# avianphysics/avian

Hardware: NVIDIA H100
Metric: physics steps/sec on 100k-cube stack (broad phase + solver stage per step) (higher is better)
Workload: dtype f32

## Files before the change

### avian_b200/csrc/broadphase.cu

```cuda
#include <algorithm>
#include <cmath>
#include <cstdlib>
#include <cstring>
#include <vector>

#include "avn_math.cuh"
#include "context.hpp"

#include "device_prims.cuh"

namespace avn {
namespace {

template <class S> struct KeyOf;
template <> struct KeyOf<float> { using type = uint32_t; static constexpr int passes = 4; };
template <> struct KeyOf<double> { using type = uint64_t; static constexpr int passes = 8; };

__device__ __forceinline__ uint32_t sortable(float f) {
    uint32_t b = __float_as_uint(f);
    if (b == 0x80000000u) b = 0;
    return (b & 0x80000000u) ? ~b : (b | 0x80000000u);
}
__device__ __forceinline__ uint64_t sortable(double f) {
    uint64_t b = (uint64_t)__double_as_longlong(f);
// ... 143 lines not shown
        if (!EMIT && threadIdx.x == 0) sub_counts[w * nsub + sub] = total;
    }
}
__global__ void wide_finish(const int* __restrict__ wide_list, const int* __restrict__ wide_count, uint32_t* __restrict__ sub_counts, int nsub,
                            uint32_t* __restrict__ counts) {
    const int nw = min(*wide_count, SW_WIDE_CAP);
    for (int w = blockIdx.x * blockDim.x + threadIdx.x; w < nw; w += gridDim.x * blockDim.x) {
        uint32_t run = 0;
        for (int k = 0; k < nsub; ++k) {
            uint32_t c = sub_counts[w * nsub + k];
            sub_counts[w * nsub + k] = run;
            run += c;
        }
        counts[wide_list[w]] = run;
    }
}

}
}
#include "broadphase_cells.cuh"
namespace avn {
namespace {

template <class S>
class Broadphase final : public BroadphaseBase {
    using K = typename KeyOf<S>::type;

   public:
    Broadphase(cudaStream_t stream, ErrorSink* err, int device) : stream_(stream), err_(err) {
        cudaDeviceProp prop;
        if (cudaGetDeviceProperties(&prop, device) == cudaSuccess) sm_count_ = prop.multiProcessorCount;
        cudaEventCreate(&ev0_);
        cudaEventCreate(&ev1_);
        cudaHostAlloc(&h_total_, 2 * sizeof(uint64_t), cudaHostAllocDefault);
        const char* g = getenv("AVN_BP_GRAPH");
        use_graph_ = !(g && !strcmp(g, "0"));
    }
    ~Broadphase() override {
        cudaEventDestroy(ev0_);
        cudaEventDestroy(ev1_);
        if (h_total_) cudaFreeHost(h_total_);
        if (graph_exec_) cudaGraphExecDestroy(graph_exec_);
    }
    AvnStatus upload(AvnAabbColumns* a) override;
    AvnStatus run() override;
    AvnStatus download(AvnPairList* out) override;
    AvnStatus device_pairs(DevicePairs* out) override;
    AvnStatus download_order(uint64_t* out_pair_count) override;
    void set_existing_device(const uint64_t* table, uint64_t mask) override { ext_existing_ = table; ext_existing_mask_ = mask; }
    void timings(AvnTimings* t) const override { *t = tm_; }

   private:
    template <class T> AvnStatus up(DevBuf& buf, const void* host, size_t count, const T** dev) {
        *dev = nullptr;
        if (!host || count == 0) return AVN_OK;
        AVN_CUDA(buf.ensure(count * sizeof(T)));
        AVN_CUDA(cudaMemcpyAsync(buf.p, host, count * sizeof(T), cudaMemcpyHostToDevice, stream_));
        *dev = buf.as<T>();
        return AVN_OK;
    }
    AvnStatus build_set(DevBuf& keys_buf, DevBuf& table_buf, const uint64_t* host_keys, uint64_t count, const uint64_t** table, uint64_t* mask);
    static constexpr int WIDE_ROWS = 64;
    uint32_t graph_replays_ = 0;
    Sweep<S> sweep_desc() const {
        Sweep<S> sw;
        sw.n = n_; sw.minx = s_minx_.as<S>(); sw.maxx = s_maxx_.as<S>(); sw.yz = s_yz_.as<Vec4<S>>(); sw.meta = s_meta_.as<uint4>();
        sw.flags = s_flags_.as<uint8_t>(); sw.end = s_end_.as<int>(); sw.is_wide = wide_flag_.as<uint8_t>();
        sw.existing = d_existing_; sw.existing_mask = existing_mask_; sw.jdis = d_jdis_; sw.jdis_mask = jdis_mask_;
        return sw;
    }
    CellSweep<S> cell_desc() const {
        CellSweep<S> cs;
        cs.grid = grid_.as<CellGrid<S>>(); cs.cranks = cv0_.as<uint32_t>(); cs.cstart = cbounds_.as<int>(); cs.cend = cbounds_.as<int>() + 0x10000;
        cs.capacity = pair_capacity_;
        return cs;
    }
    AvnStatus ensure_buffers(int n);
    void enqueue_front(int n);
    AvnStatus drop_nonfinite();
    AvnStatus settle();
    AvnStatus finish_download();
    const uint64_t* ext_existing_ = nullptr; uint64_t ext_existing_mask_ = 0;

    struct GraphKey {
        int n = -1;
        const void* p[24] = {};
        uint64_t m[2] = {};
        bool operator==(const GraphKey& o) const { return n == o.n && !memcmp(p, o.p, sizeof p) && !memcmp(m, o.m, sizeof m); }
    };
    GraphKey graph_key() const;
    bool use_graph_ = true;
    cudaGraphExec_t graph_exec_ = nullptr;
    GraphKey graph_key_{};
    uint32_t front_launches_ = 0;
    DevBuf nf_flag_;
    bool dropped_ = false;
    std::vector<uint32_t> keep_;
    std::vector<unsigned char> c_min_, c_max_;
    std::vector<uint32_t> c_col_, c_body_, c_memb_, c_filt_;
    std::vector<uint8_t> c_flags_;

    cudaStream_t stream_;
    ErrorSink* err_;
    int sm_count_ = 132;
    cudaEvent_t ev0_, ev1_;
    uint64_t* h_total_ = nullptr;
    AvnTimings tm_{};
    uint32_t launches_ = 0, upload_launches_ = 0;
    bool uploaded_ = false, ran_ = false;
    int n_ = 0;
    uint64_t pair_capacity_ = 0;
    AvnAabbColumns host_{};
    AvnAabbColumns* caller_ = nullptr;
    const S* d_min_ = nullptr; const S* d_max_ = nullptr;
    const uint32_t* d_collider_ = nullptr; const uint32_t* d_body_ = nullptr; const uint32_t* d_memb_ = nullptr; const uint32_t* d_filt_ = nullptr;
    const uint8_t* d_flags_ = nullptr;
    const uint64_t* d_existing_ = nullptr; uint64_t existing_mask_ = 0;
    const uint64_t* d_jdis_ = nullptr; uint64_t jdis_mask_ = 0;
    DevBuf b_min_, b_max_, b_col_, b_body_, b_memb_, b_filt_, b_flags_, b_exk_, b_ext_, b_jdk_, b_jdt_;
    DevBuf k0_, k1_, v0_, v1_, hist_;
    DevBuf s_minx_, s_maxx_, s_yz_, s_meta_, s_flags_, s_end_, counts_, offsets_, block_sums_, wide_, wide_sub_, wide_flag_, grid_, ck0_, ck1_, cv0_, cv1_, cbounds_, pairs_, stats_, stats2_;
    DevBuf o_c1_, o_c2_, o_b1_, o_b2_, o_fl_;
    uint32_t* d_order_ = nullptr;
};

template <class S>
AvnStatus Broadphase<S>::build_set(DevBuf& keys_buf, DevBuf& table_buf, const uint64_t* host_keys, uint64_t count, const uint64_t** table, uint64_t* mask) {
    *table = nullptr;
    *mask = 0;
    if (!host_keys || count == 0) return AVN_OK;
    uint64_t cap = 64;
    while (cap < count * 2) cap <<= 1;
    const uint64_t* dkeys;
    AvnStatus st = up<uint64_t>(keys_buf, host_keys, count, &dkeys);
    if (st != AVN_OK) return st;
// ... 57 lines not shown
    AVN_CUDA(wide_.ensure((size_t(SW_WIDE_CAP) + 1) * 4));
    AVN_CUDA(wide_flag_.ensure(size_t(n)));
    const int nsub = (n + SW_SUB - 1) / SW_SUB;
    AVN_CUDA(wide_sub_.ensure(size_t(nsub) * size_t(std::min(n, SW_WIDE_CAP)) * 4));
    AVN_CUDA(block_sums_.ensure(size_t((n + 1023) / 1024) * 8));
    AVN_CUDA(nf_flag_.ensure(8));
    pair_capacity_ = std::max<uint64_t>(pair_capacity_, uint64_t(4) * uint64_t(n) + 1024);
    AVN_CUDA(o_c1_.ensure(pair_capacity_ * 4)); AVN_CUDA(o_c2_.ensure(pair_capacity_ * 4)); AVN_CUDA(o_b1_.ensure(pair_capacity_ * 4)); AVN_CUDA(o_b2_.ensure(pair_capacity_ * 4));
    AVN_CUDA(o_fl_.ensure(pair_capacity_));
    AVN_CUDA(pairs_.ensure(pair_capacity_ * sizeof(uint2)));
    return AVN_OK;
}

template <class S>
typename Broadphase<S>::GraphKey Broadphase<S>::graph_key() const {
    GraphKey k;
    k.n = n_;
    const void* ptrs[] = {d_min_, d_max_, d_collider_, d_body_, d_memb_, d_filt_, d_flags_, d_existing_, d_jdis_, k0_.p, k1_.p, v0_.p, v1_.p, hist_.p,
                          s_minx_.p, s_maxx_.p, s_yz_.p, s_meta_.p, s_flags_.p, s_end_.p, counts_.p, offsets_.p, grid_.p, ck0_.p};
    static_assert(sizeof ptrs == sizeof k.p, "graph key size");
    memcpy(k.p, ptrs, sizeof ptrs);
    k.m[0] = existing_mask_ ^ (uint64_t(uintptr_t(cv0_.p)) << 1) ^ (uint64_t(uintptr_t(wide_sub_.p)) << 2);
    k.m[0] ^= (pair_capacity_ * 0x9e3779b97f4a7c15ull) ^ (uint64_t(uintptr_t(pairs_.p)) << 3) ^ (uint64_t(uintptr_t(o_c1_.p)) << 4) ^ (uint64_t(uintptr_t(o_fl_.p)) << 5);
    k.m[1] = jdis_mask_ ^ (uint64_t(uintptr_t(cbounds_.p)) << 1) ^ (uint64_t(uintptr_t(block_sums_.p)) << 2) ^ (uint64_t(uintptr_t(wide_flag_.p)) << 3);
    return k;
}

template <class S>
void Broadphase<S>::enqueue_front(int n) {
    const int nblocks = (n + RS_TILE - 1) / RS_TILE;
    uint32_t launches = 0;
    K* ka = k0_.as<K>(); K* kb = k1_.as<K>();
    uint32_t* va = v0_.as<uint32_t>(); uint32_t* vb = v1_.as<uint32_t>();
    cudaMemsetAsync(nf_flag_.p, 0, 8, stream_);
    make_keys<S><<<(n + 255) / 256, 256, 0, stream_>>>(d_min_, d_max_, n, ka, va, nf_flag_.as<unsigned long long>());
    ++launches;
    for (int pass = 0; pass < KeyOf<S>::passes; ++pass) {
        const int shift = 8 * pass;
        rs_histogram<K><<<nblocks, RS_THREADS, 0, stream_>>>(ka, n, shift, hist_.as<uint32_t>(), nblocks);
        if (nblocks <= RS_FUSE_MAX_BLOCKS) {
            rs_scatter<K, true><<<nblocks, RS_THREADS, 0, stream_>>>(ka, va, n, shift, hist_.as<uint32_t>(), nblocks, kb, vb);
        } else {
            rs_scan<<<1, 1024, 0, stream_>>>(hist_.as<uint32_t>(), 256 * nblocks);
            rs_scatter<K, false><<<nblocks, RS_THREADS, 0, stream_>>>(ka, va, n, shift, hist_.as<uint32_t>(), nblocks, kb, vb);
        }
        launches += nblocks <= RS_FUSE_MAX_BLOCKS ? 2 : 3;
        std::swap(ka, kb);
        std::swap(va, vb);
    }
    d_order_ = va;
    gather_sorted<S><<<(n + 255) / 256, 256, 0, stream_>>>(d_order_, n, d_min_, d_max_, d_collider_, d_body_, d_memb_, d_filt_, d_flags_,
                                                           s_minx_.as<S>(), s_maxx_.as<S>(), s_yz_.as<Vec4<S>>(), s_meta_.as<uint4>(),
                                                           s_flags_.as<uint8_t>());
    CellGrid<S>* d_grid = grid_.as<CellGrid<S>>();
    int* cstart = cbounds_.as<int>();
    int* cend = cbounds_.as<int>() + 0x10000;
    yz_stats<S><<<YZ_BLOCKS, 256, 0, stream_>>>(s_yz_.as<Vec4<S>>(), n, stats_.as<YzPartial<S>>());
    yz_fold<S><<<1, 32, 0, stream_>>>(stats_.as<YzPartial<S>>(), YZ_BLOCKS, n, d_grid);
    yz_small_max<S><<<YZ_BLOCKS, 256, 0, stream_>>>(s_yz_.as<Vec4<S>>(), n, d_grid, stats2_.as<S>());
    yz_grid<S><<<1, 32, 0, stream_>>>(stats_.as<YzPartial<S>>(), stats2_.as<S>(), YZ_BLOCKS, n, d_grid);
    int* wide_count = wide_.as<int>();
    int* wide_list = wide_.as<int>() + 1;
    cudaMemsetAsync(wide_count, 0, 4, stream_);
    sweep_bounds<S><<<(n + 255) / 256, 256, 0, stream_>>>(s_minx_.as<S>(), s_maxx_.as<S>(), s_yz_.as<Vec4<S>>(), d_grid, n, s_end_.as<int>(), wide_list, wide_count,
                                                          wide_flag_.as<uint8_t>(), s_flags_.as<uint8_t>());
    const Sweep<S> sw = sweep_desc();
    cell_keys<S><<<(n + 255) / 256, 256, 0, stream_>>>(s_yz_.as<Vec4<S>>(), n, d_grid, ck0_.as<uint32_t>(), cv0_.as<uint32_t>());
    {
        uint32_t* cka = ck0_.as<uint32_t>(); uint32_t* ckb = ck1_.as<uint32_t>();
        uint32_t* cva = cv0_.as<uint32_t>(); uint32_t* cvb = cv1_.as<uint32_t>();
        for (int pass = 0; pass < 2; ++pass) {
            rs_histogram<uint32_t><<<nblocks, RS_THREADS, 0, stream_>>>(cka, n, 8 * pass, hist_.as<uint32_t>(), nblocks);
            if (nblocks <= RS_FUSE_MAX_BLOCKS) {
                rs_scatter<uint32_t, true><<<nblocks, RS_THREADS, 0, stream_>>>(cka, cva, n, 8 * pass, hist_.as<uint32_t>(), nblocks, ckb, cvb);
            } else {
                rs_scan<<<1, 1024, 0, stream_>>>(hist_.as<uint32_t>(), 256 * nblocks);
                rs_scatter<uint32_t, false><<<nblocks, RS_THREADS, 0, stream_>>>(cka, cva, n, 8 * pass, hist_.as<uint32_t>(), nblocks, ckb, cvb);
            }
            std::swap(cka, ckb);
            std::swap(cva, cvb);
        }
    }
    cudaMemsetAsync(cstart, 0x7f, size_t(0x10000) * 4, stream_);
    cudaMemsetAsync(cend, 0, size_t(0x10000) * 4, stream_);
    cell_bounds<<<(n + 255) / 256, 256, 0, stream_>>>(ck0_.as<uint32_t>(), n, cstart, cend);
    const CellSweep<S> cs = cell_desc();
    const int grid = std::min((n + (256 / CG_GROUP) - 1) / (256 / CG_GROUP), sm_count_ * 32);
    sweep_cells_kernel<S, false><<<grid, 256, 0, stream_>>>(sw, cs, counts_.as<uint32_t>(), nullptr, nullptr);
    const int nsub = (n + SW_SUB - 1) / SW_SUB;
    sweep_wide_kernel<S, false><<<dim3(nsub, WIDE_ROWS), SW_THREADS, 0, stream_>>>(sw, wide_list, wide_count, wide_sub_.as<uint32_t>(), nsub, nullptr, nullptr, 0);
    wide_finish<<<1, 256, 0, stream_>>>(wide_list, wide_count, wide_sub_.as<uint32_t>(), nsub, counts_.as<uint32_t>());
    launches += nblocks <= RS_FUSE_MAX_BLOCKS ? 15 : 17;
    const int sblocks = (n + 1023) / 1024;
    scan_block_sums<<<sblocks, 1024, 0, stream_>>>(counts_.as<uint32_t>(), n, block_sums_.as<uint64_t>());
    scan_block_offsets<<<1, 1024, 0, stream_>>>(block_sums_.as<uint64_t>(), sblocks, offsets_.as<uint64_t>() + n);
    scan_apply<<<sblocks, 1024, 0, stream_>>>(counts_.as<uint32_t>(), n, block_sums_.as<uint64_t>(), offsets_.as<uint64_t>());
    launches += 3;
    {
        uint2* pairs = pairs_.as<uint2>();
        sweep_cells_kernel<S, true><<<grid, 256, 0, stream_>>>(sw, cs, nullptr, offsets_.as<uint64_t>(), pairs);
        sweep_wide_kernel<S, true><<<dim3(nsub, WIDE_ROWS), SW_THREADS, 0, stream_>>>(sw, wide_list, wide_count, wide_sub_.as<uint32_t>(), nsub,
                                                                                      offsets_.as<uint64_t>(), pairs, pair_capacity_);
        segment_sort<<<(n + 255) / 256, 256, 0, stream_>>>(offsets_.as<uint64_t>(), wide_flag_.as<uint8_t>(), n, pairs, pair_capacity_);
        const unsigned mblocks = unsigned(std::min<uint64_t>((pair_capacity_ + 255) / 256, uint64_t(sm_count_) * 16));
        materialize_pairs<S><<<mblocks, 256, 0, stream_>>>(sw, pairs, offsets_.as<uint64_t>() + n, pair_capacity_, o_c1_.as<uint32_t>(), o_c2_.as<uint32_t>(),
                                                           o_b1_.as<uint32_t>(), o_b2_.as<uint32_t>(), o_fl_.as<uint8_t>());
        launches += 4;
    }
    cudaMemcpyAsync(h_total_, offsets_.as<uint64_t>() + n, sizeof(uint64_t), cudaMemcpyDeviceToHost, stream_);
    cudaMemcpyAsync(h_total_ + 1, nf_flag_.p, sizeof(uint64_t), cudaMemcpyDeviceToHost, stream_);
    front_launches_ = launches;
}

template <class S>
AvnStatus Broadphase<S>::run() {
    if (!uploaded_) return err_->fail(AVN_ERR_INVALID_ARGUMENT, "avn_broadphase_run before avn_broadphase_upload");
    const int n = n_;
    launches_ = upload_launches_;
    cudaEventRecord(ev0_, stream_);
    h_total_[0] = 0;
    h_total_[1] = 0;
    if (n > 0) {
        AvnStatus st = ensure_buffers(n);
        if (st != AVN_OK) return st;
        if (use_graph_) {
            const GraphKey key = graph_key();
            if (!graph_exec_ || !(key == graph_key_)) {
                if (graph_exec_) { cudaGraphExecDestroy(graph_exec_); graph_exec_ = nullptr; }
                cudaGraph_t g = nullptr;
                AVN_CUDA(cudaStreamBeginCapture(stream_, cudaStreamCaptureModeThreadLocal));
                enqueue_front(n);
                cudaError_t ce = cudaStreamEndCapture(stream_, &g);
                if (ce == cudaSuccess) ce = cudaGraphInstantiate(&graph_exec_, g, 0);
                if (g) cudaGraphDestroy(g);
                if (ce != cudaSuccess) {
// ... 156 lines not shown
```

### avian_b200/csrc/solver_dev.cuh

```cuda
#pragma once
#include <cuda_pipeline.h>

#include "../../include/avian_b200.h"
#include "avn_math.cuh"

namespace avn {

enum { CP_N = 0, CP_T1 = 1, CP_TV = 2, CP_IDX = 3, CP_PT0 = 4, CP_PLANES = CP_PT0 + 3 * AVN_MAX_MANIFOLD_POINTS };
#define CP_ROW(k, r) (CP_PT0 + 3 * (k) + (r))
enum { CI_NP_MASK = 0x7, CI_ZERO1 = 1 << 4, CI_ZERO2 = 1 << 5, CI_NONDYN = 1 << 6, CI_TANGENT = 1 << 7,
       CI_VER1 = 1 << 8, CI_VER2 = 1 << 9 };
enum { BF_LOCK_MASK = 0x3f, BF_HAS_SOLVER_BODY = 1 << 8, BF_KINEMATIC = 1 << 9, BF_GYRO = 1 << 10, BF_DYNAMIC = 1 << 11,
       BF_CUSTOM_VEL = 1 << 12, BF_CUSTOM_POS = 1 << 13, BF_DOMINANCE_SHIFT = 16 };

enum { JP_IDX = 0,
       JP_R1 = 1,
       JP_R2 = 2,
       JP_CD = 3,
       JP_RD = 4,
       JP_A1 = 5,
       JP_A2 = 6,
       JP_B1 = 7,
       JP_B2 = 8,
       JP_LP = 9,
       JP_LA = 10,
       JP_LB = 11,
       JP_PLANES = 12 };

template <class S>
struct Soft { S bias, mass_scale, impulse_scale; };

template <class S>
struct DevSolver {
    int B, M, P, Mpad, J, Jpad, n_levels, n_damp_levels;
    int m_color_off[AVN_GRAPH_COLOR_COUNT + 1];
    int color_off[AVN_GRAPH_COLOR_COUNT + 1];
    int color_len[AVN_GRAPH_COLOR_COUNT];
    int wave;
    unsigned int* ver;
    int* deg;
    int* stamp;
    int substeps, iters, rest_iters, fast_trig, match_contacts;
    S h, dt, max_overlap_speed, warm_coeff, rest_threshold, joint_force_rhs;
    S gx, gy, gz;
    Soft<S> soft_dyn, soft_nondyn;
    const uint8_t* kind; const uint8_t* locked; const int8_t* dominance; const uint8_t* integ_flags;
    const S* position; const S* rotation; const S* linvel; const S* angvel; const S* inv_mass; const S* inv_inertia_local;
    const S* com; const S* lin_damp; const S* ang_damp; const S* grav_scale; const S* lin_acc; const S* ang_acc;
    const S* max_lin; const S* max_ang;
    S* out_position; S* out_rotation; S* out_linvel; S* out_angvel;
    Vec4<S>* vel; Vec4<S>* dlt; Vec4<S>* inr; Vec4<S>* itg; Vec4<S>* pre;
    const int* m_body1; const int* m_body2; const S* m_normal; const S* m_friction; const S* m_restitution; const S* m_tanvel;
    const uint32_t* m_point_begin; const uint32_t* m_point_end; const uint32_t* m_src;
    const S* p_anchor1; const S* p_anchor2; const S* p_penetration; const S* p_normal_speed;
    const S* p_ws_normal; const S* p_ws_tangent;
    const S* p_in_normal_impulse;
    S* p_out_ws_normal; S* p_out_ws_tangent; S* p_normal_impulse;
    Vec4<S>* cst;
    Vec4<S>* pcr;
    int* any_restitution;
    const int* j_src_type; const int* j_src_index;
    const int* level_off;
    Vec4<S>* jnt;
    const S* jc[AVN_JOINT_TYPE_COUNT][12];
    const S* jdamp_lin[AVN_JOINT_TYPE_COUNT]; const S* jdamp_ang[AVN_JOINT_TYPE_COUNT];
    const uint8_t* jlimit_en[AVN_JOINT_TYPE_COUNT]; const uint8_t* jdamp_en[AVN_JOINT_TYPE_COUNT];
    const int* jbody1[AVN_JOINT_TYPE_COUNT]; const int* jbody2[AVN_JOINT_TYPE_COUNT];
    S* jforce[AVN_JOINT_TYPE_COUNT]; S* jtorque[AVN_JOINT_TYPE_COUNT];
    const int* jdamp_slot; const int* damp_level_off;
    Vec4<S>* jdummy;
    int do_prepare, sub_begin, sub_end, do_restitution, do_finalize;
    const int* bnd_of;
    Vec4<S>* vel_ref;
};
// ... 593 lines not shown
        st4(&d.vel[2 * b2 + 1], mk4<S>(w2.x, w2.y, w2.z, S(0)));
    }
    wave_publish(d.ver, ver1, b1, e1, ver2, b2, e2);
#ifdef AVN_WAVE_TRACE
    AVN_TRACE_ADD(d, 3, clock64() - t_s0);
    AVN_TRACE_ADD(d, 4, 1);
#endif
#undef ROW_A
#undef ROW_B
#undef ROW_D
#undef ROW_PC
}

template <class S, bool WAVE = false>
__device__ __forceinline__ void integrate_velocity_item(const DevSolver<S>& d, int i, int s = 0) {
    const bool in_range = i < d.B;
    int f = 0;
    if (in_range) f = as_int(ld4(&d.inr[2 * i]).y);
    const bool live = in_range && (f & BF_HAS_SOLVER_BODY);
    const bool integrate = live && !(f & BF_CUSTOM_VEL) && !(f & BF_KINEMATIC), gyro = integrate && (f & BF_GYRO);
    Vec4<S> li = mk4<S>(0, 0, 0, 0), ai = li;
    Q4<S> rot0; rot0.x = rot0.y = rot0.z = rot0.w = S(0);
    Sym3<S> il; il.m00 = il.m01 = il.m02 = il.m11 = il.m12 = il.m22 = S(0);
    if (integrate) { li = ld4(&d.itg[2 * i]); ai = ld4(&d.itg[2 * i + 1]); }
    if (gyro) {
        rot0 = ldq(d.rotation, i);
        il.m00 = d.inv_inertia_local[6 * i]; il.m01 = d.inv_inertia_local[6 * i + 1]; il.m02 = d.inv_inertia_local[6 * i + 2];
        il.m11 = d.inv_inertia_local[6 * i + 3]; il.m12 = d.inv_inertia_local[6 * i + 4]; il.m22 = d.inv_inertia_local[6 * i + 5];
    }
    const S max_lin = live && d.max_lin ? d.max_lin[i] : S(0), max_ang = live && d.max_ang ? d.max_ang[i] : S(0);
    const int bnd = live && d.bnd_of ? d.bnd_of[i] : -1;
    unsigned e = 0;
    if (WAVE) {
        if (live) e = wave_event(WV_IV, 0, s, d.iters, d.deg[i], 0);
        wave_wait(d.ver, live, i, e, false, 0, 0u, d.any_restitution + 1);
    }
    if (!live) return;
    Vec4<S> l = ldm<WAVE>(&d.vel[2 * i]), a = ldm<WAVE>(&d.vel[2 * i + 1]);
    V3<S> v = xyz(l), w = xyz(a);
    bool touched = false;
    if (integrate) {
        v = v * li.w;
        w = w * ai.w;
        v = v + xyz(li);
        w = w + xyz(ai);
        if (gyro) {
            Vec4<S> dq4 = ldm<WAVE>(&d.dlt[2 * i + 1]);
            Q4<S> dq; dq.x = dq4.x; dq.y = dq4.y; dq.z = dq4.z; dq.w = dq4.w;
            Q4<S> rot = qmul(dq, rot0);
            V3<S> lw = qrot(qconj(rot), w);
            Sym3<S> tensor = sym_inverse_or_zero(il);
            V3<S> L = smul(tensor, lw);
            V3<S> Ln = L - d.h * cross(lw, L);
            S l2 = len2(Ln);
            if (l2 == S(0)) {
                w = zero3<S>();
            } else {
                Ln = Ln * avn_sqrt(len2(L) / l2);
                w = qrot(rot, smul(il, Ln));
            }
        }
        touched = true;
    }
    if (d.max_lin) {
        S l2 = len2(v);
        if (avn_finite(max_lin) && l2 > max_lin * max_lin) { v = v * (max_lin / avn_sqrt(l2)); touched = true; }
    }
    if (d.max_ang) {
        S l2 = len2(w);
        if (avn_finite(max_ang) && l2 > max_ang * max_ang) { w = w * (max_ang / avn_sqrt(l2)); touched = true; }
    }
    if (touched) {
        st4(&d.vel[2 * i], mk4<S>(v.x, v.y, v.z, S(0)));
        st4(&d.vel[2 * i + 1], mk4<S>(w.x, w.y, w.z, S(0)));
    }
    if (bnd >= 0) {
        st4(&d.vel_ref[2 * bnd], mk4<S>(v.x, v.y, v.z, S(0)));
        st4(&d.vel_ref[2 * bnd + 1], mk4<S>(w.x, w.y, w.z, S(0)));
    }
    if (WAVE) wave_publish(d.ver, true, i, e, false, 0, 0u);
}

template <class S, bool WAVE = false>
__device__ __forceinline__ void integrate_position_item(const DevSolver<S>& d, int i, int s = 0) {
    const bool in_range = i < d.B;
    int f = 0;
    if (in_range) f = as_int(ld4(&d.inr[2 * i]).y);
    const bool live = in_range && (f & BF_HAS_SOLVER_BODY);
    unsigned e = 0;
    if (WAVE) {
        if (live) e = wave_event(WV_IP, 0, s, d.iters, d.deg[i], 0);
        wave_wait(d.ver, live, i, e, false, 0, 0u, d.any_restitution + 1);
    }
    if (!live) return;
    if (f & BF_CUSTOM_POS) {
        if (WAVE) wave_publish(d.ver, true, i, e, false, 0, 0u);
        return;
    }
    Vec4<S> l = ldm<WAVE>(&d.vel[2 * i]), a = ldm<WAVE>(&d.vel[2 * i + 1]);
    Vec4<S> dp = ldm<WAVE>(&d.dlt[2 * i]), dq4 = ldm<WAVE>(&d.dlt[2 * i + 1]);
    V3<S> ndp = xyz(dp) + xyz(l) * d.h;
    Q4<S> dq; dq.x = dq4.x; dq.y = dq4.y; dq.z = dq4.z; dq.w = dq4.w;
    Q4<S> nq = qmul(q_from_scaled_axis(xyz(a) * d.h, d.fast_trig != 0), dq);
    st4(&d.dlt[2 * i], mk4<S>(ndp.x, ndp.y, ndp.z, S(0)));
    st4(&d.dlt[2 * i + 1], mk4<S>(nq.x, nq.y, nq.z, nq.w));
    if (WAVE) wave_publish(d.ver, true, i, e, false, 0, 0u);
}

enum { WAVE_WATCHDOG = 1, WAVE_BAD_COLOURING = 3 };
template <class S>
__device__ __forceinline__ void wave_rank_item(const DevSolver<S>& d, int slot) {
    const size_t MP = size_t(d.Mpad);
    Vec4<S>* c = d.cst + slot;
    Vec4<S> hidx = ld4(&c[CP_IDX * MP]);
    const int info = as_int(hidx.z);
    if ((info & CI_NP_MASK) == 0) return;
    const int b1 = as_int(hidx.x), b2 = as_int(hidx.y);
    int colour = 0;
    while (colour < AVN_GRAPH_COLOR_COUNT - 1 && slot >= d.color_off[colour + 1]) ++colour;
    int r1 = 0, r2 = 0;
    bool bad = false;
    if (info & CI_VER1) { bad |= atomicExch(&d.stamp[b1], colour + 1) == colour + 1; r1 = atomicAdd(&d.deg[b1], 1); }
    if (info & CI_VER2) { bad |= atomicExch(&d.stamp[b2], colour + 1) == colour + 1; r2 = atomicAdd(&d.deg[b2], 1); }
    if (bad || r1 > 0xfe || r2 > 0xfe) d.any_restitution[1] = WAVE_BAD_COLOURING;
    hidx.w = int_as(S(0), (r1 & 0xff) | ((r2 & 0xff) << 16));
    st4(&c[CP_IDX * MP], hidx);
}
template <class S>
__device__ __forceinline__ void wave_pack_item(const DevSolver<S>& d, int slot) {
    const size_t MP = size_t(d.Mpad);
    Vec4<S>* c = d.cst + slot;
    Vec4<S> hidx = ld4(&c[CP_IDX * MP]);
    const int info = as_int(hidx.z);
    if ((info & CI_NP_MASK) == 0) return;
    const int b1 = as_int(hidx.x), b2 = as_int(hidx.y);
    int rk = as_int(hidx.w);
    if (info & CI_VER1) rk |= (d.deg[b1] & 0xff) << 8;
    if (info & CI_VER2) rk |= (d.deg[b2] & 0xff) << 24;
    hidx.w = int_as(S(0), rk);
    st4(&c[CP_IDX * MP], hidx);
}

template <class S>
__device__ __forceinline__ void writeback_body_item(const DevSolver<S>& d, int i) {
    Vec4<S> ia = ld4(&d.inr[2 * i]);
    int f = as_int(ia.y);
    V3<S> pos = ldv3(d.position, i);
    Q4<S> rot = ldq(d.rotation, i);
    V3<S> lv = ldv3(d.linvel, i), av = ldv3(d.angvel, i);
    if (f & BF_HAS_SOLVER_BODY) {
        Vec4<S> l = ld4(&d.vel[2 * i]), a = ld4(&d.vel[2 * i + 1]);
        Vec4<S> dp = ld4(&d.dlt[2 * i]), dq4 = ld4(&d.dlt[2 * i + 1]);
        V3<S> com = ldv3_or0(d.com, i);
        V3<S> old_com = qrot(rot, com);
        Q4<S> dq; dq.x = dq4.x; dq.y = dq4.y; dq.z = dq4.z; dq.w = dq4.w;
        rot = q_fast_renormalize(qmul(dq, rot));
        V3<S> new_com = qrot(rot, com);
        pos = pos + ((xyz(dp) + old_com) - new_com);
        lv = xyz(l);
        av = xyz(a);
    }
    stv3(d.out_position, i, pos);
    d.out_rotation[4 * i] = rot.x; d.out_rotation[4 * i + 1] = rot.y; d.out_rotation[4 * i + 2] = rot.z; d.out_rotation[4 * i + 3] = rot.w;
    stv3(d.out_linvel, i, lv);
    stv3(d.out_angvel, i, av);
}

template <class S>
__device__ __forceinline__ void store_impulse_item(const DevSolver<S>& d, int m) {
    const size_t MP = size_t(d.Mpad);
    const int slot = slot_of_manifold(d, m);
// ... 23 lines not shown
```

### avian_b200/csrc/solver_host.cu

```cuda
#include <algorithm>
#include <cmath>
#include <cstdlib>
#include <cstring>

#include "context.hpp"
#include "joint_schedule.hpp"
#include "solver_kernels.cuh"

namespace avn {

namespace {

template <class S>
Soft<S> softness(S damping_ratio, S hz, S delta_secs) {
    S double_damping_ratio = S(2) * damping_ratio;
    S angular_frequency = S(6.283185307179586476925286766559) * hz;
    S a1 = double_damping_ratio + angular_frequency * delta_secs;
    S a2 = angular_frequency * delta_secs * a1;
    S a3 = S(1) / (S(1) + a2);
    Soft<S> s;
    s.bias = angular_frequency / a1;
    s.mass_scale = a2 * a3;
    s.impulse_scale = a3;
    return s;
// ... 446 lines not shown
            d.p_ws_normal = static_cast<const S*>(mc->ws_normal); d.p_ws_tangent = static_cast<const S*>(mc->ws_tangent);
            d.p_in_normal_impulse = static_cast<const S*>(mc->normal_impulse);
            d.p_out_ws_normal = static_cast<S*>(mc->out_ws_normal); d.p_out_ws_tangent = static_cast<S*>(mc->out_ws_tangent);
            d.p_normal_impulse = static_cast<S*>(mc->out_normal_impulse);
            host_any_restitution_ = mc->list_restitution;
        } else {
            UP(m_b1_, mc->body1, M, int, m_body1);
            UP(m_b2_, mc->body2, M, int, m_body2);
            UP(m_f_, mc->friction, M, S, m_friction);
            UP(m_r_, mc->restitution, M, S, m_restitution);
            UP(m_n_, mc->normal, 3 * M, S, m_normal);
            UP(m_tv_, mc->tangent_velocity, 3 * M, S, m_tanvel);
            UP(m_po_, mc->point_offsets, M + 1, uint32_t, m_point_begin);
            d.m_point_end = d.m_point_begin + 1;
            UP(p_a1_, mc->anchor1, 3 * P, S, p_anchor1);
            UP(p_a2_, mc->anchor2, 3 * P, S, p_anchor2);
            UP(p_pen_, mc->penetration, P, S, p_penetration);
            UP(p_ns_, mc->normal_speed, P, S, p_normal_speed);
            UP(p_wn_, mc->ws_normal, P, S, p_ws_normal);
            UP(p_wt_, mc->ws_tangent, 2 * P, S, p_ws_tangent);
            UP(p_nin_, mc->normal_impulse, P, S, p_in_normal_impulse);
            AVN_CUDA(p_own_.ensure(P * sizeof(S) + 16)); d.p_out_ws_normal = p_own_.as<S>();
            AVN_CUDA(p_owt_.ensure(2 * P * sizeof(S) + 16)); d.p_out_ws_tangent = p_owt_.as<S>();
            AVN_CUDA(p_ni_.ensure(P * sizeof(S) + 16));
            d.p_normal_impulse = p_ni_.as<S>();
            host_any_restitution_ = false;
            const S* r = static_cast<const S*>(mc->restitution);
            for (size_t i = 0; i < M; ++i) host_any_restitution_ |= (r[i] != S(0));
        }
        hm_ = *mc;
    }
    {
        auto up256 = [](size_t x) { return (x + 255) & ~size_t(255); };
        const size_t vel_b = up256(state_bytes), dlt_b = up256(state_bytes), ver_b = up256((B + 1) * sizeof(unsigned)), deg_b = up256(2 * (B + 1) * sizeof(int));
        const size_t planes_b = have_m_ ? size_t(CP_PLANES) * d.Mpad * sizeof(Vec4<S>) : 0;
        const size_t pcr_b = have_m_ ? up256(size_t(AVN_MAX_MANIFOLD_POINTS) * d.Mpad * sizeof(Vec4<S>)) : 0;
        AVN_CUDA(hot_.ensure(vel_b + dlt_b + ver_b + deg_b + pcr_b + planes_b + 256));
        char* base = hot_.as<char>();
        d.vel = reinterpret_cast<Vec4<S>*>(base); base += vel_b;
        d.dlt = reinterpret_cast<Vec4<S>*>(base); base += dlt_b;
        d.ver = reinterpret_cast<unsigned*>(base); base += ver_b;
        d.deg = reinterpret_cast<int*>(base); d.stamp = d.deg + (B + 1); base += deg_b;
        d.pcr = have_m_ ? reinterpret_cast<Vec4<S>*>(base) : nullptr; base += pcr_b;
        d.cst = have_m_ ? reinterpret_cast<Vec4<S>*>(base) : nullptr;
        hot_bytes_ = vel_b + dlt_b + ver_b + deg_b + pcr_b;
    }
    have_j_ = false;
    if (js) {
        size_t J = 0;
        for (int t = 0; t < AVN_JOINT_TYPE_COUNT; ++t) J += js->types[t].count;
        if (J > 0) {
            if ((st = build_joint_schedule(*bc, *js)) != AVN_OK) return st;
            have_j_ = true;
            for (int t = 0; t < AVN_JOINT_TYPE_COUNT; ++t) {
                const AvnJointColumns& jc = js->types[t];
                const size_t n = jc.count;
                const void* cols[12] = {jc.local_anchor1, jc.local_anchor2, jc.local_basis1, jc.local_basis2, jc.axis, jc.limit_min,
                                        jc.limit_max, jc.limit2_min, jc.limit2_max, jc.compliance0, jc.compliance1, jc.compliance2};
                const size_t width[12] = {3, 3, 4, 4, 3, 1, 1, 1, 1, 1, 1, 1};
                for (int c = 0; c < 12; ++c) UP(jcol_[t][c], cols[c], width[c] * n, S, jc[t][c]);
                UP(jb1_[t], jc.body1, n, int, jbody1[t]);
                UP(jb2_[t], jc.body2, n, int, jbody2[t]);
                UP(jle_[t], jc.limit_enabled, n, uint8_t, jlimit_en[t]);
                UP(jde_[t], jc.damping_enabled, n, uint8_t, jdamp_en[t]);
                UP(jdl_[t], jc.damping_linear, n, S, jdamp_lin[t]);
                UP(jda_[t], jc.damping_angular, n, S, jdamp_ang[t]);
                d.jforce[t] = nullptr;
                d.jtorque[t] = nullptr;
                if (n && jc.force) { AVN_CUDA(jfo_[t].ensure(3 * n * sizeof(S))); d.jforce[t] = jfo_[t].as<S>(); }
                if (n && jc.torque) { AVN_CUDA(jto_[t].ensure(3 * n * sizeof(S))); d.jtorque[t] = jto_[t].as<S>(); }
            }
            UP(j_type_, h_type_.data(), h_type_.size(), int, j_src_type);
            UP(j_index_, h_index_.data(), h_index_.size(), int, j_src_index);
            UP(j_level_, h_level_off_.data(), h_level_off_.size(), int, level_off);
            UP(j_damp_slot_, h_damp_slot_.data(), h_damp_slot_.size(), int, jdamp_slot);
            UP(j_damp_level_, h_damp_level_off_.data(), h_damp_level_off_.size(), int, damp_level_off);
            AVN_CUDA(j_dummy_.ensure(2 * AVN_JOINT_TYPE_COUNT * sizeof(Vec4<S>)));
            d.jdummy = j_dummy_.as<Vec4<S>>();
// ... 39 lines not shown
template <class S>
AvnStatus Solver<S>::run_range(uint32_t first, uint32_t count, uint32_t flags) {
    if (ccd_active()) return err_->fail(AVN_ERR_UNSUPPORTED, "avn_solver_run_range: swept CCD is configured (avn_solver_run runs the split step itself)");
    return launch_range(first, count, flags);
}

template <class S>
AvnStatus Solver<S>::launch_range(uint32_t first, uint32_t count, uint32_t flags) {
    if (!uploaded_) return err_->fail(AVN_ERR_INVALID_ARGUMENT, "avn_solver_run before avn_solver_upload");
    const bool prepare = (flags & AVN_RUN_PREPARE) != 0;
    if (!prepare && !prepared_) return err_->fail(AVN_ERR_INVALID_ARGUMENT, "avn_solver_run_range: the first launch after an upload must include AVN_RUN_PREPARE");
    if (uint64_t(first) + count > uint64_t(dev_.substeps)) return err_->fail(AVN_ERR_INVALID_ARGUMENT, "avn_solver_run_range: substeps [%u, %u) exceed %d", first, first + count, dev_.substeps);
    dev_.do_prepare = prepare ? 1 : 0;
    dev_.sub_begin = int(first);
    dev_.sub_end = int(first + count);
    dev_.do_restitution = (flags & AVN_RUN_RESTITUTION) ? 1 : 0;
    dev_.do_finalize = (flags & AVN_RUN_FINALIZE) ? 1 : 0;
    bool mega = use_mega_ && coop_ok_;
    if (prepare) step_bps_ = mega_bps_;
    mega = mega && select_megakernel(max_np_, step_bps_);
    if (prepare) {
        launches_ = 0;
        cudaEventRecord(ev_[EV_RUN0], stream_);
        AVN_CUDA(cudaMemsetAsync(dev_.any_restitution, 0, FLAG_WORDS * sizeof(int) + 8 * sizeof(unsigned long long), stream_));
        int widest_colour = 0;
        for (int c = 0; c < AVN_COLOR_OVERFLOW; ++c) widest_colour = std::max(widest_colour, dev_.color_len[c]);
        const bool chain_bound = force_wave_ || widest_colour <= 2 * mega_grid_ * MEGA_BLOCK;
        dev_.wave = (mega && use_wave_ && chain_bound && dev_.M > 0 && dev_.J == 0 && dev_.color_len[AVN_COLOR_OVERFLOW] == 0) ? 1 : 0;
        if (dev_.M > 0) {
            AVN_CUDA(cudaMemsetAsync(dev_.cst + size_t(CP_IDX) * dev_.Mpad, 0, size_t(dev_.Mpad) * sizeof(Vec4<S>), stream_));
        }
        if (dev_.wave) {
            AVN_CUDA(cudaMemsetAsync(dev_.ver, 0, (size_t(dev_.B) + 1) * sizeof(unsigned), stream_));
            AVN_CUDA(cudaMemsetAsync(dev_.deg, 0, 2 * (size_t(dev_.B) + 1) * sizeof(int), stream_));
        }
        mega_step_ = mega;
    } else {
        mega = mega && mega_step_;
    }
    if (l2_persist_ && hot_bytes_ > 0) {
        cudaStreamAttrValue attr{};
        attr.accessPolicyWindow.base_ptr = hot_.p;
        attr.accessPolicyWindow.num_bytes = std::min(hot_bytes_, l2_window_max_);
        attr.accessPolicyWindow.hitRatio = float(std::min(1.0, double(l2_persist_bytes_) / double(attr.accessPolicyWindow.num_bytes)));
        attr.accessPolicyWindow.hitProp = cudaAccessPropertyPersisting;
        attr.accessPolicyWindow.missProp = cudaAccessPropertyStreaming;
        cudaStreamSetAttribute(stream_, cudaStreamAttributeAccessPolicyWindow, &attr);
    }
    const DevSolver<S>& d = dev_;
    if (mega) {
        void* args[] = {(void*)&dev_};
        cudaError_t e = cudaLaunchCooperativeKernel(mega_fn_, dim3(mega_grid_), dim3(MEGA_BLOCK), args, mega_smem_bytes(mega_maxp_), stream_);
        if (e != cudaSuccess) {
            (void)cudaGetLastError();
            if (!prepare && dev_.wave)
                return err_->fail(AVN_ERR_CUDA, "cooperative launch refused in the middle of a wavefront-scheduled step: %s", cudaGetErrorString(e));
            mega = false;
            mega_step_ = false;
            dev_.wave = 0;
        } else {
            ++launches_;
            if (prepare) cudaEventRecord(ev_[EV_PREP], stream_);
            if (dev_.do_finalize) cudaEventRecord(ev_[EV_LOOP], stream_);
        }
    }
    if (!mega) {
        if (prepare) {
// ... 292 lines not shown
```

### avian_b200/csrc/solver_kernels.cuh

```cuda
#pragma once
#include <cooperative_groups.h>

#include "joints_dev.cuh"

namespace avn {
namespace cg = cooperative_groups;

constexpr int MEGA_BLOCK = 128;

enum PhaseOp {
    OP_PREPARE_BODY = 0, OP_PREPARE_CONSTRAINT, OP_PREPARE_JOINT, OP_INTEGRATE_VEL, OP_INTEGRATE_POS, OP_WARM, OP_SOLVE_BIAS,
    OP_RELAX, OP_RESTITUTION, OP_SOLVE_JOINT, OP_PROJECT_VEL, OP_DAMP_JOINT, OP_WRITEBACK_BODY, OP_STORE_IMPULSE, OP_JOINT_FORCE,
    OP_WAVE_RANK, OP_WAVE_PACK
};

template <class S, int OP, int MAXP = AVN_MAX_MANIFOLD_POINTS>
__device__ __forceinline__ void run_item(const DevSolver<S>& d, int i) {
    if (OP == OP_PREPARE_BODY) prepare_body_item(d, i);
    else if (OP == OP_PREPARE_CONSTRAINT) prepare_constraint_item(d, i);
    else if (OP == OP_PREPARE_JOINT) prepare_joint_item(d, i);
    else if (OP == OP_INTEGRATE_VEL) integrate_velocity_item(d, i);
    else if (OP == OP_INTEGRATE_POS) { integrate_position_item(d, i); if (d.J > 0) store_pre_solve_item(d, i); }
    else if (OP == OP_WARM) contact_item<S, PASS_WARM, MAXP>(d, i);
    else if (OP == OP_SOLVE_BIAS) contact_item<S, PASS_SOLVE_BIAS, MAXP>(d, i);
// ... 69 lines not shown
    const long long per_substep = (long long)first_chunks + body_chunks + (long long)(front_passes + 1) * slot_chunks;
    const long long total = per_substep * d.sub_end;
    for (long long g = per_substep * d.sub_begin + warp_id; g < total; g += warps) {
        const int s = int(g / per_substep);
        long long r = g - (long long)s * per_substep;
        if (r < first_chunks) {
            wave_iv_chunk<S, BPS, MAXP>(d, int(r) * WAVE_CHUNK + lane, s);
            continue;
        }
        r -= first_chunks;
        if (r < (long long)front_passes * slot_chunks) {
            const int pass = int(r / slot_chunks), slot = int(r - (long long)pass * slot_chunks) * WAVE_CHUNK + lane;
            if (pass == 0) wave_contact_chunk<S, PASS_WARM, MAXP, BPS>(d, slot, s, 0, false);
            else wave_contact_chunk<S, PASS_SOLVE_BIAS, MAXP, BPS>(d, slot, s, pass - 1, false);
            continue;
        }
        r -= (long long)front_passes * slot_chunks;
        if (r < body_chunks) { wave_ip_chunk<S, BPS, MAXP>(d, int(r) * WAVE_CHUNK + lane, s); continue; }
        r -= body_chunks;
        wave_contact_chunk<S, PASS_SOLVE_BIAS, MAXP, BPS>(d, int(r) * WAVE_CHUNK + lane, s, 0, true);
    }
}

template <class S, int BPS, int MAXP>
__global__ void __launch_bounds__(MEGA_BLOCK, BPS) step_megakernel(const __grid_constant__ DevSolver<S> d) {
    cg::grid_group grid = cg::this_grid();
    if (d.do_prepare) {
        grid_phase<S, OP_PREPARE_BODY>(d, 0, d.B + 1);
        grid.sync();
        grid_phase<S, OP_PREPARE_CONSTRAINT>(d, 0, d.M);
        grid_phase<S, OP_PREPARE_JOINT>(d, 0, d.J);
        grid.sync();
        if (d.wave) {
            for (int c = 0; c < AVN_COLOR_OVERFLOW; ++c) {
                if (d.color_len[c] <= 0) continue;
                grid_phase<S, OP_WAVE_RANK>(d, d.color_off[c], d.color_len[c]);
                grid.sync();
            }
            grid_phase<S, OP_WAVE_PACK>(d, 0, d.Mpad);
            grid.sync();
        }
    }
    const bool wave = d.wave && *reinterpret_cast<volatile int*>(d.any_restitution + 1) == 0;
    if (wave && d.sub_end > d.sub_begin) {
        wave_substep_loop<S, MAXP, BPS>(d);
        grid.sync();
    }
    for (int sub = d.sub_begin; sub < (wave ? 0 : d.sub_end); ++sub) {
        grid_phase<S, OP_INTEGRATE_VEL>(d, 0, d.B);
        grid.sync();
        if (d.M > 0) {
            grid_contact_pass<S, OP_WARM, MAXP>(d, grid);
            for (int it = 0; it < d.iters; ++it) grid_contact_pass<S, OP_SOLVE_BIAS, MAXP>(d, grid);
        }
        grid_phase<S, OP_INTEGRATE_POS>(d, 0, d.B);
        grid.sync();
        if (d.M > 0) grid_contact_pass<S, OP_RELAX, MAXP>(d, grid);
        if (d.J > 0) {
            for (int l = 0; l < d.n_levels; ++l) {
                const int b = d.level_off[l], n = d.level_off[l + 1] - b;
                grid_phase<S, OP_SOLVE_JOINT>(d, b, n);
                grid.sync();
            }
            grid_phase<S, OP_PROJECT_VEL>(d, 0, d.B);
            grid.sync();
            for (int l = 0; l < d.n_damp_levels; ++l) {
                const int b = d.damp_level_off[l], n = d.damp_level_off[l + 1] - b;
                grid_phase<S, OP_DAMP_JOINT>(d, b, n);
                grid.sync();
            }
        }
// ... 11 lines not shown
```

Measured before the change: 441.4.

## Overlap broadphase wide sweeps on side stream; replace per-colour rank syncs with colour bitmasks

Broadphase now forks a non-blocking side stream so the cell-bound memsets, sweep_bounds and the wide sweep kernels run concurrently with the radix sort and cell sweep on the main stream, joined by events. In the solver megakernel, per-body degree/stamp counters that needed a grid sync after each colour are replaced by a per-body bitmask of colours, set with atomicOr. Rank and degree are then derived with popc during pack, so the rank phase needs only one grid sync. The cost is extra event and stream management, which adds graph complexity, and the bitmask caps the colour count at 32.

```diff
diff --git a/avian_b200/csrc/broadphase.cu b/avian_b200/csrc/broadphase.cu
--- a/avian_b200/csrc/broadphase.cu
+++ b/avian_b200/csrc/broadphase.cu
@@ -199,6 +199,9 @@
         if (cudaGetDeviceProperties(&prop, device) == cudaSuccess) sm_count_ = prop.multiProcessorCount;
         cudaEventCreate(&ev0_);
         cudaEventCreate(&ev1_);
+        cudaStreamCreateWithFlags(&side_, cudaStreamNonBlocking);
+        cudaEventCreateWithFlags(&ev_fork_, cudaEventDisableTiming);
+        cudaEventCreateWithFlags(&ev_join_, cudaEventDisableTiming);
         cudaHostAlloc(&h_total_, 2 * sizeof(uint64_t), cudaHostAllocDefault);
         const char* g = getenv("AVN_BP_GRAPH");
         use_graph_ = !(g && !strcmp(g, "0"));
@@ -206,6 +209,9 @@
     ~Broadphase() override {
         cudaEventDestroy(ev0_);
         cudaEventDestroy(ev1_);
+        cudaEventDestroy(ev_fork_);
+        cudaEventDestroy(ev_join_);
+        cudaStreamDestroy(side_);
         if (h_total_) cudaFreeHost(h_total_);
         if (graph_exec_) cudaGraphExecDestroy(graph_exec_);
     }
@@ -268,6 +274,10 @@
     std::vector<uint8_t> c_flags_;
 
     cudaStream_t stream_;
+    cudaStream_t side_ = nullptr;
+    cudaEvent_t ev_fork_ = nullptr, ev_join_ = nullptr;
+    void fork() { cudaEventRecord(ev_fork_, stream_); cudaStreamWaitEvent(side_, ev_fork_, 0); }
+    void join() { cudaEventRecord(ev_join_, side_); cudaStreamWaitEvent(stream_, ev_join_, 0); }
     ErrorSink* err_;
     int sm_count_ = 132;
     cudaEvent_t ev0_, ev1_;
@@ -391,6 +401,11 @@
     uint32_t launches = 0;
     K* ka = k0_.as<K>(); K* kb = k1_.as<K>();
     uint32_t* va = v0_.as<uint32_t>(); uint32_t* vb = v1_.as<uint32_t>();
+    int* cstart = cbounds_.as<int>();
+    int* cend = cbounds_.as<int>() + 0x10000;
+    fork();
+    cudaMemsetAsync(cstart, 0x7f, size_t(0x10000) * 4, side_);
+    cudaMemsetAsync(cend, 0, size_t(0x10000) * 4, side_);
     cudaMemsetAsync(nf_flag_.p, 0, 8, stream_);
     make_keys<S><<<(n + 255) / 256, 256, 0, stream_>>>(d_min_, d_max_, n, ka, va, nf_flag_.as<unsigned long long>());
     ++launches;
@@ -412,17 +427,16 @@
                                                            s_minx_.as<S>(), s_maxx_.as<S>(), s_yz_.as<Vec4<S>>(), s_meta_.as<uint4>(),
                                                            s_flags_.as<uint8_t>());
     CellGrid<S>* d_grid = grid_.as<CellGrid<S>>();
-    int* cstart = cbounds_.as<int>();
-    int* cend = cbounds_.as<int>() + 0x10000;
     yz_stats<S><<<YZ_BLOCKS, 256, 0, stream_>>>(s_yz_.as<Vec4<S>>(), n, stats_.as<YzPartial<S>>());
     yz_fold<S><<<1, 32, 0, stream_>>>(stats_.as<YzPartial<S>>(), YZ_BLOCKS, n, d_grid);
     yz_small_max<S><<<YZ_BLOCKS, 256, 0, stream_>>>(s_yz_.as<Vec4<S>>(), n, d_grid, stats2_.as<S>());
     yz_grid<S><<<1, 32, 0, stream_>>>(stats_.as<YzPartial<S>>(), stats2_.as<S>(), YZ_BLOCKS, n, d_grid);
     int* wide_count = wide_.as<int>();
     int* wide_list = wide_.as<int>() + 1;
-    cudaMemsetAsync(wide_count, 0, 4, stream_);
-    sweep_bounds<S><<<(n + 255) / 256, 256, 0, stream_>>>(s_minx_.as<S>(), s_maxx_.as<S>(), s_yz_.as<Vec4<S>>(), d_grid, n, s_end_.as<int>(), wide_list, wide_count,
-                                                          wide_flag_.as<uint8_t>(), s_flags_.as<uint8_t>());
+    fork();
+    cudaMemsetAsync(wide_count, 0, 4, side_);
+    sweep_bounds<S><<<(n + 255) / 256, 256, 0, side_>>>(s_minx_.as<S>(), s_maxx_.as<S>(), s_yz_.as<Vec4<S>>(), d_grid, n, s_end_.as<int>(), wide_list, wide_count,
+                                                        wide_flag_.as<uint8_t>(), s_flags_.as<uint8_t>());
     const Sweep<S> sw = sweep_desc();
     cell_keys<S><<<(n + 255) / 256, 256, 0, stream_>>>(s_yz_.as<Vec4<S>>(), n, d_grid, ck0_.as<uint32_t>(), cv0_.as<uint32_t>());
     {
@@ -440,14 +454,15 @@
             std::swap(cva, cvb);
         }
     }
-    cudaMemsetAsync(cstart, 0x7f, size_t(0x10000) * 4, stream_);
-    cudaMemsetAsync(cend, 0, size_t(0x10000) * 4, stream_);
+    join();
     cell_bounds<<<(n + 255) / 256, 256, 0, stream_>>>(ck0_.as<uint32_t>(), n, cstart, cend);
     const CellSweep<S> cs = cell_desc();
     const int grid = std::min((n + (256 / CG_GROUP) - 1) / (256 / CG_GROUP), sm_count_ * 32);
+    const int nsub = (n + SW_SUB - 1) / SW_SUB;
+    fork();
+    sweep_wide_kernel<S, false><<<dim3(nsub, WIDE_ROWS), SW_THREADS, 0, side_>>>(sw, wide_list, wide_count, wide_sub_.as<uint32_t>(), nsub, nullptr, nullptr, 0);
     sweep_cells_kernel<S, false><<<grid, 256, 0, stream_>>>(sw, cs, counts_.as<uint32_t>(), nullptr, nullptr);
-    const int nsub = (n + SW_SUB - 1) / SW_SUB;
-    sweep_wide_kernel<S, false><<<dim3(nsub, WIDE_ROWS), SW_THREADS, 0, stream_>>>(sw, wide_list, wide_count, wide_sub_.as<uint32_t>(), nsub, nullptr, nullptr, 0);
+    join();
     wide_finish<<<1, 256, 0, stream_>>>(wide_list, wide_count, wide_sub_.as<uint32_t>(), nsub, counts_.as<uint32_t>());
     launches += nblocks <= RS_FUSE_MAX_BLOCKS ? 15 : 17;
     const int sblocks = (n + 1023) / 1024;
@@ -457,9 +472,11 @@
     launches += 3;
     {
         uint2* pairs = pairs_.as<uint2>();
+        fork();
+        sweep_wide_kernel<S, true><<<dim3(nsub, WIDE_ROWS), SW_THREADS, 0, side_>>>(sw, wide_list, wide_count, wide_sub_.as<uint32_t>(), nsub,
+                                                                                    offsets_.as<uint64_t>(), pairs, pair_capacity_);
         sweep_cells_kernel<S, true><<<grid, 256, 0, stream_>>>(sw, cs, nullptr, offsets_.as<uint64_t>(), pairs);
-        sweep_wide_kernel<S, true><<<dim3(nsub, WIDE_ROWS), SW_THREADS, 0, stream_>>>(sw, wide_list, wide_count, wide_sub_.as<uint32_t>(), nsub,
-                                                                                      offsets_.as<uint64_t>(), pairs, pair_capacity_);
+        join();
         segment_sort<<<(n + 255) / 256, 256, 0, stream_>>>(offsets_.as<uint64_t>(), wide_flag_.as<uint8_t>(), n, pairs, pair_capacity_);
         const unsigned mblocks = unsigned(std::min<uint64_t>((pair_capacity_ + 255) / 256, uint64_t(sm_count_) * 16));
         materialize_pairs<S><<<mblocks, 256, 0, stream_>>>(sw, pairs, offsets_.as<uint64_t>() + n, pair_capacity_, o_c1_.as<uint32_t>(), o_c2_.as<uint32_t>(),
diff --git a/avian_b200/csrc/solver_dev.cuh b/avian_b200/csrc/solver_dev.cuh
--- a/avian_b200/csrc/solver_dev.cuh
+++ b/avian_b200/csrc/solver_dev.cuh
@@ -38,8 +38,7 @@
     int color_len[AVN_GRAPH_COLOR_COUNT];
     int wave;
     unsigned int* ver;
-    int* deg;
-    int* stamp;
+    unsigned* mask;
     int substeps, iters, rest_iters, fast_trig, match_contacts;
     S h, dt, max_overlap_speed, warm_coeff, rest_threshold, joint_force_rhs;
     S gx, gy, gz;
@@ -699,7 +698,7 @@
     const int bnd = live && d.bnd_of ? d.bnd_of[i] : -1;
     unsigned e = 0;
     if (WAVE) {
-        if (live) e = wave_event(WV_IV, 0, s, d.iters, d.deg[i], 0);
+        if (live) e = wave_event(WV_IV, 0, s, d.iters, __popc(d.mask[i]), 0);
         wave_wait(d.ver, live, i, e, false, 0, 0u, d.any_restitution + 1);
     }
     if (!live) return;
@@ -756,7 +755,7 @@
     const bool live = in_range && (f & BF_HAS_SOLVER_BODY);
     unsigned e = 0;
     if (WAVE) {
-        if (live) e = wave_event(WV_IP, 0, s, d.iters, d.deg[i], 0);
+        if (live) e = wave_event(WV_IP, 0, s, d.iters, __popc(d.mask[i]), 0);
         wave_wait(d.ver, live, i, e, false, 0, 0u, d.any_restitution + 1);
     }
     if (!live) return;
@@ -776,22 +775,21 @@
 
 enum { WAVE_WATCHDOG = 1, WAVE_BAD_COLOURING = 3 };
 template <class S>
+__device__ __forceinline__ int wave_slot_colour(const DevSolver<S>& d, int slot) {
+    int colour = 0;
+    while (colour < AVN_GRAPH_COLOR_COUNT - 1 && slot >= d.color_off[colour + 1]) ++colour;
+    return colour;
+}
+template <class S>
 __device__ __forceinline__ void wave_rank_item(const DevSolver<S>& d, int slot) {
-    const size_t MP = size_t(d.Mpad);
-    Vec4<S>* c = d.cst + slot;
-    Vec4<S> hidx = ld4(&c[CP_IDX * MP]);
+    const Vec4<S> hidx = ld4(&d.cst[CP_IDX * size_t(d.Mpad) + slot]);
     const int info = as_int(hidx.z);
     if ((info & CI_NP_MASK) == 0) return;
-    const int b1 = as_int(hidx.x), b2 = as_int(hidx.y);
-    int colour = 0;
-    while (colour < AVN_GRAPH_COLOR_COUNT - 1 && slot >= d.color_off[colour + 1]) ++colour;
-    int r1 = 0, r2 = 0;
+    const unsigned bit = 1u << wave_slot_colour(d, slot);
     bool bad = false;
-    if (info & CI_VER1) { bad |= atomicExch(&d.stamp[b1], colour + 1) == colour + 1; r1 = atomicAdd(&d.deg[b1], 1); }
-    if (info & CI_VER2) { bad |= atomicExch(&d.stamp[b2], colour + 1) == colour + 1; r2 = atomicAdd(&d.deg[b2], 1); }
-    if (bad || r1 > 0xfe || r2 > 0xfe) d.any_restitution[1] = WAVE_BAD_COLOURING;
-    hidx.w = int_as(S(0), (r1 & 0xff) | ((r2 & 0xff) << 16));
-    st4(&c[CP_IDX * MP], hidx);
+    if (info & CI_VER1) bad |= (atomicOr(&d.mask[as_int(hidx.x)], bit) & bit) != 0;
+    if (info & CI_VER2) bad |= (atomicOr(&d.mask[as_int(hidx.y)], bit) & bit) != 0;
+    if (bad) d.any_restitution[1] = WAVE_BAD_COLOURING;
 }
 template <class S>
 __device__ __forceinline__ void wave_pack_item(const DevSolver<S>& d, int slot) {
@@ -800,10 +798,10 @@
     Vec4<S> hidx = ld4(&c[CP_IDX * MP]);
     const int info = as_int(hidx.z);
     if ((info & CI_NP_MASK) == 0) return;
-    const int b1 = as_int(hidx.x), b2 = as_int(hidx.y);
-    int rk = as_int(hidx.w);
-    if (info & CI_VER1) rk |= (d.deg[b1] & 0xff) << 8;
-    if (info & CI_VER2) rk |= (d.deg[b2] & 0xff) << 24;
+    const unsigned below = (1u << wave_slot_colour(d, slot)) - 1u;
+    int rk = 0;
+    if (info & CI_VER1) { const unsigned m = d.mask[as_int(hidx.x)]; rk |= __popc(m & below) | (__popc(m) << 8); }
+    if (info & CI_VER2) { const unsigned m = d.mask[as_int(hidx.y)]; rk |= (__popc(m & below) << 16) | (__popc(m) << 24); }
     hidx.w = int_as(S(0), rk);
     st4(&c[CP_IDX * MP], hidx);
 }
diff --git a/avian_b200/csrc/solver_host.cu b/avian_b200/csrc/solver_host.cu
--- a/avian_b200/csrc/solver_host.cu
+++ b/avian_b200/csrc/solver_host.cu
@@ -502,18 +502,18 @@
     }
     {
         auto up256 = [](size_t x) { return (x + 255) & ~size_t(255); };
-        const size_t vel_b = up256(state_bytes), dlt_b = up256(state_bytes), ver_b = up256((B + 1) * sizeof(unsigned)), deg_b = up256(2 * (B + 1) * sizeof(int));
+        const size_t vel_b = up256(state_bytes), dlt_b = up256(state_bytes), ver_b = up256((B + 1) * sizeof(unsigned)), mask_b = up256((B + 1) * sizeof(unsigned));
         const size_t planes_b = have_m_ ? size_t(CP_PLANES) * d.Mpad * sizeof(Vec4<S>) : 0;
         const size_t pcr_b = have_m_ ? up256(size_t(AVN_MAX_MANIFOLD_POINTS) * d.Mpad * sizeof(Vec4<S>)) : 0;
-        AVN_CUDA(hot_.ensure(vel_b + dlt_b + ver_b + deg_b + pcr_b + planes_b + 256));
+        AVN_CUDA(hot_.ensure(vel_b + dlt_b + ver_b + mask_b + pcr_b + planes_b + 256));
         char* base = hot_.as<char>();
         d.vel = reinterpret_cast<Vec4<S>*>(base); base += vel_b;
         d.dlt = reinterpret_cast<Vec4<S>*>(base); base += dlt_b;
         d.ver = reinterpret_cast<unsigned*>(base); base += ver_b;
-        d.deg = reinterpret_cast<int*>(base); d.stamp = d.deg + (B + 1); base += deg_b;
+        d.mask = reinterpret_cast<unsigned*>(base); base += mask_b;
         d.pcr = have_m_ ? reinterpret_cast<Vec4<S>*>(base) : nullptr; base += pcr_b;
         d.cst = have_m_ ? reinterpret_cast<Vec4<S>*>(base) : nullptr;
-        hot_bytes_ = vel_b + dlt_b + ver_b + deg_b + pcr_b;
+        hot_bytes_ = vel_b + dlt_b + ver_b + mask_b + pcr_b;
     }
     have_j_ = false;
     if (js) {
@@ -619,7 +619,7 @@
         }
         if (dev_.wave) {
             AVN_CUDA(cudaMemsetAsync(dev_.ver, 0, (size_t(dev_.B) + 1) * sizeof(unsigned), stream_));
-            AVN_CUDA(cudaMemsetAsync(dev_.deg, 0, 2 * (size_t(dev_.B) + 1) * sizeof(int), stream_));
+            AVN_CUDA(cudaMemsetAsync(dev_.mask, 0, (size_t(dev_.B) + 1) * sizeof(unsigned), stream_));
         }
         mega_step_ = mega;
     } else {
diff --git a/avian_b200/csrc/solver_kernels.cuh b/avian_b200/csrc/solver_kernels.cuh
--- a/avian_b200/csrc/solver_kernels.cuh
+++ b/avian_b200/csrc/solver_kernels.cuh
@@ -125,11 +125,9 @@
         grid_phase<S, OP_PREPARE_JOINT>(d, 0, d.J);
         grid.sync();
         if (d.wave) {
-            for (int c = 0; c < AVN_COLOR_OVERFLOW; ++c) {
-                if (d.color_len[c] <= 0) continue;
-                grid_phase<S, OP_WAVE_RANK>(d, d.color_off[c], d.color_len[c]);
-                grid.sync();
-            }
+            for (int c = 0; c < AVN_COLOR_OVERFLOW; ++c)
+                if (d.color_len[c] > 0) grid_phase<S, OP_WAVE_RANK>(d, d.color_off[c], d.color_len[c]);
+            grid.sync();
             grid_phase<S, OP_WAVE_PACK>(d, 0, d.Mpad);
             grid.sync();
         }
```

Result: faster. 448.1 (median of 6 runs) (+1.5%).
